# NekoImageLand/retto

Measured on AMD Instinct MI355X. Metric: images/sec end-to-end PP-OCRv4 det+rec @960x960, higher is better.
Workload: dtype f32

## Files before the change

### include/retto_hip.h

```cpp
#ifndef RETTO_HIP_H
#define RETTO_HIP_H

#include <stddef.h>
#include <stdint.h>

#ifdef __cplusplus
extern "C" {
#endif

#define RT_API __attribute__((visibility("default")))

typedef enum rt_status {
  RT_OK = 0,
  RT_ERR_IO = 1,
  RT_ERR_IMAGE = 2,
  RT_ERR_SHAPE = 3,
  RT_ERR_BACKEND = 4,
  RT_ERR_UTF8 = 5,
  RT_ERR_MODEL_NOT_FOUND = 7,
  RT_ERR_INVALID = 8,
  RT_ERR_CAPACITY = 9
} rt_status;

typedef struct rt_model_source {
// ... 69 lines not shown
                        int mem, const float* const* det_map_override, rt_results** out);
typedef void (*rt_stage_callback)(void* user, int page, int stage, const char* json);
RT_API int rt_run_batch_stream(rt_session* s, const uint8_t* const* rgb, const int* hs, const int* ws, int n_pages,
                               int mem, const float* const* det_map_override, rt_stage_callback cb, void* user,
                               rt_results** out);
#define RT_MAX_INFLIGHT 8
typedef struct rt_ticket rt_ticket;
RT_API int rt_submit_batch(rt_session* s, const uint8_t* const* rgb, const int* hs, const int* ws, int n_pages, int mem,
                           const float* const* det_map_override, rt_ticket** out);
RT_API int rt_wait_batch(rt_session* s, rt_ticket* ticket, rt_results** out);
RT_API void rt_results_free(rt_results* r);
RT_API int rt_results_pages(const rt_results* r);
RT_API int rt_results_count(const rt_results* r, int page);
RT_API const float* rt_results_boxes(const rt_results* r, int page);
RT_API const float* rt_results_det_scores(const rt_results* r, int page);
RT_API const uint16_t* rt_results_cls_labels(const rt_results* r, int page);
RT_API const float* rt_results_cls_scores(const rt_results* r, int page);
RT_API const float* rt_results_rec_scores(const rt_results* r, int page);
RT_API int rt_results_rec_tokens(const rt_results* r, int page, int line, const int32_t** tokens);
RT_API const char* rt_results_rec_text(const rt_results* r, int page, int line);
RT_API double rt_results_det_checksum(const rt_results* r);
RT_API const char* rt_results_json(rt_results* r, int page, int stage);

RT_API int rt_device_malloc(rt_session* s, size_t bytes, void** out);
RT_API int rt_device_free(rt_session* s, void* p);
RT_API int rt_memcpy_h2d(rt_session* s, void* dst, const void* src, size_t bytes);
RT_API int rt_memcpy_d2h(rt_session* s, void* dst, const void* src, size_t bytes);
RT_API int rt_synchronize(rt_session* s);
RT_API int rt_set_lanes(rt_session* s, int lanes);
RT_API int rt_profile_enable(rt_session* s, int on);
RT_API int rt_profile_get(rt_session* s, const char* const** names, const float** ms, const int** calls, int* n);

RT_API int rt_onnx_to_rtwb(int which, const void* onnx, size_t len, void** out, size_t* out_len, char* err, size_t err_cap);
RT_API void rt_buffer_free(void* p);

RT_API int rt_host_cpu_budget(void);
RT_API int rt_decode_image(const void* data, size_t len, uint8_t** rgb, int* h, int* w, char* err, size_t err_cap);
RT_API int rt_run_encoded_batch(rt_session* s, const void* const* files, const size_t* lens, int n_pages,
                                rt_stage_callback cb, void* user, rt_results** out);
RT_API int rt_parse_dictionary(const void* data, size_t len, char** out, size_t* out_len, int* n_entries, char* err, size_t err_cap);
RT_API int rt_format_f32(float v, char* buf, size_t cap);
RT_API size_t rt_model_manifest(int which, char* buf, size_t cap);

RT_API int rt_rccl_unique_id(void* id, size_t cap, char* err, size_t err_cap);
RT_API int rt_broadcast_blobs(const void* id, int rank, int world, int device_id, int root, int n_blobs, void** data, size_t* lens,
                              char* err, size_t err_cap);

RT_API void rt_debug_set_variants(int gemm_variant, int dw_variant, int flags);
RT_API int rt_debug_conv16(rt_session* s, const float* x, int n, int cin, int h, int w, const float* wt, int cout, int kh, int kw,
                           int sh, int sw, const float* bias, int act, float* out);
RT_API int rt_bench_gemm(rt_session* s, long long M, int K, int N, int variant, int iters, float* ms_out, float* maxdiff_out);
RT_API int rt_bench_gemm_err(rt_session* s, long long M, int K, int N, int variant, int rows, int act, unsigned seed, double* out4);
RT_API int rt_bench_lc(rt_session* s, int n, int h, int w, int cin, int cout, int stride, int form, int iters, float* ms_out, float* maxdiff_out);

#ifdef __cplusplus
}
#endif
#endif
```

### retto_amd/_lib.py

```python
from __future__ import annotations

import ctypes as C
import os

_HERE = os.path.dirname(os.path.abspath(__file__))
LIB_PATH = os.path.join(_HERE, "libretto_hip.so")

RT_OK = 0
RT_MEM_HOST, RT_MEM_DEVICE, RT_MEM_HOST_MAPS_DEVICE = 0, 1, 2
RT_MAX_INFLIGHT = 8
RT_DTYPE_F32, RT_DTYPE_F16 = 0, 1
STATUS_NAMES = {0: "OK", 1: "IOError", 2: "ImageError", 3: "ShapeError", 4: "BackendError", 5: "Utf8Error",
                7: "ModelNotFoundError", 8: "InvalidArgument", 9: "CapacityError"}


class ModelSource(C.Structure):
    _fields_ = [("path", C.c_char_p), ("data", C.c_void_p), ("len", C.c_size_t)]


class Config(C.Structure):
    _fields_ = [
        ("struct_size", C.c_uint32), ("device_id", C.c_int32),
        ("det", ModelSource), ("cls", ModelSource), ("rec", ModelSource), ("dict", ModelSource),
        ("max_side_len", C.c_int32), ("min_side_len", C.c_int32),
        ("det_limit_side_len", C.c_int32), ("det_limit_type", C.c_int32),
        ("det_mean", C.c_float * 3), ("det_std", C.c_float * 3), ("det_scale", C.c_float),
        ("det_thresh", C.c_float), ("det_box_thresh", C.c_float), ("det_unclip_ratio", C.c_float),
        ("det_min_mini_box_size", C.c_int32), ("det_dilation", C.c_int32),
        ("cls_image_shape", C.c_int32 * 3), ("cls_batch_num", C.c_int32), ("cls_thresh", C.c_float),
        ("rec_image_shape", C.c_int32 * 3), ("rec_batch_num", C.c_int32),
        ("max_boxes_per_page", C.c_int32), ("det_sub_batch", C.c_int32), ("lanes", C.c_int32), ("dtype", C.c_int32),
    ]


EXPORTS = [
    "rt_config_default", "rt_create", "rt_destroy", "rt_last_error", "rt_version",
    "rt_det", "rt_cls", "rt_rec", "rt_rec_ragged", "rt_rec_classes", "rt_model_info",
    "rt_resize_both_dims", "rt_resize_both", "rt_det_input_dims", "rt_det_preprocess", "rt_det_postprocess",
    "rt_crop_dims", "rt_crop_images", "rt_scale_and_clip", "rt_resize_norm_width", "rt_resize_norm_image",
    "rt_ctc_decode",
    "rt_run_batch", "rt_run_batch_stream", "rt_submit_batch", "rt_wait_batch", "rt_host_cpu_budget", "rt_results_free", "rt_results_pages", "rt_results_count", "rt_results_boxes",
    "rt_results_det_scores", "rt_results_cls_labels", "rt_results_cls_scores", "rt_results_rec_scores",
    "rt_results_rec_tokens", "rt_results_rec_text", "rt_results_det_checksum", "rt_results_json",
    "rt_device_malloc", "rt_device_free", "rt_memcpy_h2d", "rt_memcpy_d2h", "rt_synchronize",
    "rt_set_lanes", "rt_profile_enable", "rt_profile_get",
    "rt_onnx_to_rtwb", "rt_buffer_free", "rt_model_manifest", "rt_decode_image", "rt_run_encoded_batch",
    "rt_debug_set_variants", "rt_bench_gemm", "rt_bench_gemm_err", "rt_bench_lc", "rt_debug_conv16", "rt_parse_dictionary", "rt_format_f32", "rt_rccl_unique_id", "rt_broadcast_blobs",
]

STAGE_CALLBACK = C.CFUNCTYPE(None, C.c_void_p, C.c_int, C.c_int, C.c_char_p)

_lib = None


def source_digest() -> str:
    import glob
    import hashlib
    h = hashlib.sha256()
    files = sorted(glob.glob(os.path.join(_HERE, "csrc", "*.hip")) + glob.glob(os.path.join(_HERE, "csrc", "*.cpp")) +
                   glob.glob(os.path.join(_HERE, "csrc", "*.h")) + [os.path.join(os.path.dirname(_HERE), "include", "retto_hip.h")])
    for f in files:
        h.update(os.path.basename(f).encode()); h.update(open(f, "rb").read())
    return h.hexdigest()[:16]


def load():
    global _lib
    if _lib is not None:
        return _lib
    if not os.path.exists(LIB_PATH):
        raise ImportError(
            f"{LIB_PATH} is missing: build it with `make -C retto_amd/csrc` (python -c 'import __graft_entry__ as g; "
            "g.build()'). retto_amd has no CPU fallback.")
    lib = C.CDLL(LIB_PATH)
    P = C.POINTER
    lib.rt_last_error.restype = C.c_char_p
    lib.rt_last_error.argtypes = [C.c_void_p]
    lib.rt_version.restype = C.c_char_p
    lib.rt_create.argtypes = [P(Config), P(C.c_void_p)]
    lib.rt_destroy.argtypes = [C.c_void_p]
    lib.rt_destroy.restype = None
    lib.rt_results_free.argtypes = [C.c_void_p]
    lib.rt_results_free.restype = None
    lib.rt_results_boxes.restype = P(C.c_float)
    lib.rt_results_det_scores.restype = P(C.c_float)
    lib.rt_results_cls_labels.restype = P(C.c_uint16)
    lib.rt_results_cls_scores.restype = P(C.c_float)
    lib.rt_results_rec_scores.restype = P(C.c_float)
    lib.rt_results_rec_text.restype = C.c_char_p
    lib.rt_results_json.restype = C.c_char_p
    lib.rt_results_det_checksum.restype = C.c_double
    for name in ("rt_results_boxes", "rt_results_det_scores", "rt_results_cls_labels", "rt_results_cls_scores",
                 "rt_results_rec_scores", "rt_results_count"):
        getattr(lib, name).argtypes = [C.c_void_p, C.c_int]
    lib.rt_results_pages.argtypes = [C.c_void_p]
    lib.rt_results_det_checksum.argtypes = [C.c_void_p]
    lib.rt_results_rec_tokens.argtypes = [C.c_void_p, C.c_int, C.c_int, P(P(C.c_int32))]
    lib.rt_results_rec_text.argtypes = [C.c_void_p, C.c_int, C.c_int]
    lib.rt_results_json.argtypes = [C.c_void_p, C.c_int, C.c_int]
    lib.rt_scale_and_clip.argtypes = [C.c_void_p, C.c_int, C.c_double, C.c_double, C.c_double, C.c_double]
# ... 43 lines not shown
```

### retto_amd/csrc/api.cpp

```cpp
#include <thread>
#include <sched.h>
#include <atomic>
#include <cmath>
#include <cstdio>
#include <cstdlib>
#include <cstring>
#include <new>

#include "geom_math.h"
#include "session.h"
#include "onnx_import.h"
#include "image_decode.h"

using namespace rt;

static thread_local std::string g_create_error;
static void capture_variant_defaults();
const char* rt_results_json_impl(rt_results* r, int page, int stage);

static void quiesce(rt_session* s) {
  if (!s) return;
  (void)hipSetDevice(s->device);
  if (s->st) (void)hipStreamSynchronize(s->st);
  for (auto& h : s->helpers)
// ... 613 lines not shown
    float *dx = bufs.alloc<float>(nin), *dwd = bufs.alloc<float>(hwd.size()), *dbd = bufs.alloc<float>(hbd.size()), *dw = bufs.alloc<float>(hw.size()),
          *db = bufs.alloc<float>(hb.size()), *dy = bufs.alloc<float>(nout), *dy0 = bufs.alloc<float>(nout);
    ImgGeom *dgi = bufs.alloc<ImgGeom>(n), *dgo = bufs.alloc<ImgGeom>(n);
    RT_HIP_CHECK(hipMemset(dy, 0, nout * 4)); RT_HIP_CHECK(hipMemset(dy0, 0, nout * 4));
    RT_HIP_CHECK(hipMemcpy(dx, hx.data(), nin * 4, hipMemcpyHostToDevice)); RT_HIP_CHECK(hipMemcpy(dwd, hwd.data(), hwd.size() * 4, hipMemcpyHostToDevice));
    RT_HIP_CHECK(hipMemcpy(dbd, hbd.data(), hbd.size() * 4, hipMemcpyHostToDevice)); RT_HIP_CHECK(hipMemcpy(dw, hw.data(), hw.size() * 4, hipMemcpyHostToDevice));
    RT_HIP_CHECK(hipMemcpy(db, hb.data(), hb.size() * 4, hipMemcpyHostToDevice));
    RT_HIP_CHECK(hipMemcpy(dgi, gi.data(), n * sizeof(ImgGeom), hipMemcpyHostToDevice)); RT_HIP_CHECK(hipMemcpy(dgo, go.data(), n * sizeof(ImgGeom), hipMemcpyHostToDevice));
    Epilogue e; e.bias = db; e.act = ACT_HSWISH; e.has_lab = 1; e.lab_a = 1.01f; e.lab_c = 0.02f;
    const int dw_act = (sh == 2 && sw == 2) ? ACT_NONE : ACT_HSWISH, dw_lab = !(sh == 2 && sw == 2);
    float* dy1 = nullptr;
    auto run = [&](float* out) {
      if (nn::g_lc_wave == 0 && !nn::lc_thin_supported(3, sh, sw, Cp, cin, Np)) {
        if (!dy1) dy1 = bufs.alloc<float>((size_t)n * ho * wo * Cp);
        nn::dwconv(s->st, 3, sh, sw, dx, dgi, dgo, n, ho, wo, Cp, cin, dwd, dbd, dw_act, dw_lab, 0.99f, 0.01f, dy1, nullptr);
        nn::gemm(s->st, dy1, Cp, (long long)n * ho * wo, Cp, dw, cout, Np, out, ldy, 0, e);
        return;
      }
      nn::lc_thin(s->st, sh, sw, dx, dgi, dgo, n, ho, wo, Cp, cin, dwd, dbd, dw_act, dw_lab, 0.99f, 0.01f, dw, cout, Np, out, ldy, e);
    };
    nn::g_lc_wave = getenv("RT_BENCH_LC_REF") ? atoi(getenv("RT_BENCH_LC_REF")) : 0; run(dy0);
    nn::g_lc_wave = form; run(dy);
    Events ev; RT_HIP_CHECK(hipEventCreate(&ev.a)); RT_HIP_CHECK(hipEventCreate(&ev.b));
    hipEvent_t a = ev.a, b = ev.b;
    RT_HIP_CHECK(hipEventRecord(a, s->st));
    for (int i = 0; i < iters; i++) run(dy);
    RT_HIP_CHECK(hipEventRecord(b, s->st));
    RT_HIP_CHECK(hipStreamSynchronize(s->st));
    float ms = 0; RT_HIP_CHECK(hipEventElapsedTime(&ms, a, b)); *ms_out = ms / iters;
    if (maxdiff_out) {
      const size_t cnt = std::min<size_t>(nout, (size_t)1 << 22);
      std::vector<float> c0(cnt), c1(cnt);
      float md = 0;
      for (size_t off : {(size_t)0, nout - cnt}) {
        RT_HIP_CHECK(hipMemcpy(c0.data(), dy0 + off, cnt * 4, hipMemcpyDeviceToHost)); RT_HIP_CHECK(hipMemcpy(c1.data(), dy + off, cnt * 4, hipMemcpyDeviceToHost));
        size_t bad = 0;
        std::map<std::string, int> hist;
        for (size_t i = 0; i < cnt; i++) {
          const float d = std::fabs(c0[i] - c1[i]); md = (d > md || d != d) ? (d != d ? INFINITY : d) : md;
          if (d != 0 && getenv("RT_BENCH_LC_DUMP")) {
            const size_t e = off + i, px = e / ldy; const int ch = (int)(e % ldy), img = (int)(px / ((size_t)ho * wo)), yy = (int)(px % ((size_t)ho * wo)) / wo, xx = (int)(px % wo);
            if (bad++ < 4) fprintf(stderr, "  diff img %d y %d x %d ch %d: %g vs %g\n", img, yy, xx, ch, c0[i], c1[i]);
            hist["x%16=" + std::to_string(xx % 16)]++; hist["ch%4=" + std::to_string(ch % 4)]++; hist["ch/16=" + std::to_string(ch / 16)]++; hist["y%2=" + std::to_string(yy % 2)]++;
            hist["tx=" + std::to_string(xx / 16)]++; hist["q=" + std::to_string((ch % 16) / 4)]++;
          }
        }
        if (bad) { fprintf(stderr, "  %zu of %zu differ:", bad, cnt); for (auto& kv : hist) fprintf(stderr, " %s:%d", kv.first.c_str(), kv.second); fprintf(stderr, "\n"); }
      }
      *maxdiff_out = md;
    }
  });
}

}
```

### retto_amd/csrc/nn.h

```cpp
#pragma once
#include "common.h"

namespace rt {
namespace nn {

constexpr int KC = 32;

void gemm(hipStream_t st, const float* A, int lda, long long M, int K, const float* Wp, int N, int Npad16, float* C,
          int ldc, int coff, const Epilogue& epi);
const char* gemm_pw_label(long long M, int Npad16, bool a_scale = false, int se_tile_rows = 0);
bool gemm_w_supported(int lda, long long M, int K, int N, int Npad16, const Epilogue& epi, int ldc = 0, int coff = 0);
void gemm_w(hipStream_t st, const float* A, int lda, long long M, int K, const float* Wp, int N, int Npad16, float* C, int ldc, int coff,
            const Epilogue& epi);
bool gemm_dma_supported(int lda, long long M, int K, int N, int Npad16, const Epilogue& epi);
void gemm_dma(hipStream_t st, const float* A, int lda, long long M, int K, const float* Wp, int N, int Npad16, float* C,
              int ldc, int coff, const Epilogue& epi);
extern int g_gemm_split;
bool gemm_split_supported(int lda, long long M, int K, int N, int Npad16, const Epilogue& epi);
void gemm_split(hipStream_t st, const float* A, int lda, long long M, int K, const float* Wp, int N, int Npad16, float* C,
                int ldc, int coff, const Epilogue& epi);
void gemm_split_forget(const float* Wp);
void set_dw_xcd(int v);
extern int g_dw_wide_slab_min, g_dw_wide3_min, g_dw_wide_lp;
extern int g_dw_variant;
extern int g_gemm_variant;
extern int g_gemm_dma;
extern int g_dw_sweep;

bool conv13_flat_supported(int N, int Npad16);
void conv13_flat(hipStream_t st, const float* x, int ldx, long long rows, const unsigned char* flags, int Cin, const float* Wp, int N,
                 int Npad16, float* y, int ldy, const Epilogue& epi);
void conv_sp(hipStream_t st, int KH, int KW, const float* x, int ldx, const ImgGeom* geom, int n_img, int maxH,
             int maxW, int Cin, const float* Wp, int N, int Npad16, float* y, int ldy, const Epilogue& epi);

void dwconv(hipStream_t st, int K, int sh, int sw, const float* x, const ImgGeom* gin, const ImgGeom* gout, int n_img,
            int maxHo, int maxWo, int Cp, int C, const float* Wd, const float* bias, int act, int has_lab,
            float lab_a, float lab_c, float* y, float* pool = nullptr);
void dwconv_pool_layout(int K, int sh, int sw, int Cp, int maxHo, int maxWo, int* chunks, int* strip_R, int* strips_per_block);
void se_fc_from_dw(hipStream_t st, const float* partial, const ImgGeom* geom, int n_img, int chunks, int strip_R,
                   int strips_per_block, int C, int Cp, const float* w1, const float* b1, const float* w2, const float* b2,
                   int Cr, float slope, int residual, float* scale);
int gemm_tile_rows(long long M, int Npad16);
int gemm_se_tile_rows(int lda, long long M, int K, int N, int Npad16, int act, long long min_pix);
extern int g_argmax_wide;
int gemm_argmax_tiles(int Npad16);
void argmax_merge(hipStream_t st, const float* pm, const int* pi, const float* ps, int tiles, long long rows, int* idx,
                  float* prob);

extern int g_cls_fused;
bool cls_block_supported(int k, int sh, int sw, int cin, int mid, int cout, int act, int maxH_in, int maxW, int max_pix_out);
void cls_block(hipStream_t st, int k, int sh, bool se, int act, const float* x, const ImgGeom* gin, const ImgGeom* gout, int n_img,
               int maxH_in, int maxW, int max_pix_out, int cin, int mid, int mid_cp, int cout, const float* Wexp, const float* bexp,
               const float* Wdw, const float* bdw, const float* w1, const float* b1, const float* w2, const float* b2, int cr, float slope,
               const float* Wlin, const float* blin, bool shortcut, float* y, float* dscr);
extern int g_lc_thin;
bool lc_thin_supported(int K, int sh, int sw, int Cp, int C, int Npad16);
void lc_thin(hipStream_t st, int sh, int sw, const float* x, const ImgGeom* gin, const ImgGeom* gout, int n_img, int maxHo,
             int maxWo, int Cp, int C, const float* Wd, const float* bd, int dw_act, int dw_has_lab, float dw_a, float dw_c,
             const float* Wp, int N, int Npad16, float* y, int ldy, const Epilogue& epi);
extern int g_lc_wave;
bool lc_block_supported(int K, int sh, int sw, int Cp, int C, int N, int Npad16, int dw_act, int dw_has_lab, const Epilogue& epi,
                        int maxHo, int maxWo);
bool lc_wave_supported(int K, int sh, int sw, int Cp, int C, int N, int Npad16, int dw_act, int dw_has_lab, const Epilogue& epi);
void lc_wave(hipStream_t st, int sh, int sw, const float* x, const ImgGeom* gin, const ImgGeom* gout, int n_img, int maxHo,
             int maxWo, int Cp, int C, const float* Wd, const float* bd, int dw_act, int dw_has_lab, float dw_a, float dw_c,
             const float* Wp, int N, int Npad16, float* y, int ldy, const Epilogue& epi);

struct U8Page { const uint8_t* rgb; long long npix; long long out_pix; };
void stem_conv_u8(hipStream_t st, const U8Page* pages, float scale, const float* mean3, const float* std3, const ImgGeom* gin,
                  const ImgGeom* gout, int n_img, int maxHo, int maxWo, int COUT, const float* Ws, const float* bias, int act,
                  float* y);
void stem_conv(hipStream_t st, const float* x, const ImgGeom* gin, const ImgGeom* gout, int n_img, int maxHo, int maxWo,
               int COUT, const float* Ws, const float* bias, int act, float* y);

void nchw3_to_nhwc4(hipStream_t st, const float* in, int n, int H, int W, float* out);

int pool_chunks(long long max_pix);
void se_scale(hipStream_t st, const float* x, const ImgGeom* geom, int n_img, long long max_pix, int C, int Cp,
              const float* w1, const float* b1, const float* w2, const float* b2, int Cr, float slope, int residual,
              float* partial, float* scale);
// ... 62 lines not shown
```

### retto_amd/csrc/nn_kernels.hip

```cpp
#include "nn.h"
#include "nn_dev.h"

#include <algorithm>
#include <cstdlib>

namespace rt {
namespace nn {

constexpr int LROW = KC + 4;

template <int NT>
__device__ __forceinline__ void mma_chunk(const float* __restrict__ xs0, const float* __restrict__ xs1,
                                          const float* __restrict__ ws, int nt_valid, f32x4 (&acc)[2][NT], int r,
                                          int q) {
#pragma unroll
  for (int g = 0; g < KC / 16; g++) {
    f32x4 a0 = *reinterpret_cast<const f32x4*>(xs0 + g * 16 + 4 * q);
    f32x4 a1 = *reinterpret_cast<const f32x4*>(xs1 + g * 16 + 4 * q);
#pragma unroll
    for (int nt = 0; nt < NT; nt++) {
      if (nt < nt_valid) {
        f32x4 b = *reinterpret_cast<const f32x4*>(ws + (nt * 16 + r) * LROW + g * 16 + 4 * q);
#pragma unroll
        for (int s = 0; s < 4; s++) {
// ... 1227 lines not shown
#pragma unroll
      for (int dx = 0; dx < K; dx++) {
        const f32x4 w = *reinterpret_cast<const f32x4*>(wl + ((dy * K + dx) * LP + c4) * 4);
#pragma unroll
        for (int j = 0; j < 4; j++)
#pragma unroll
          for (int e = 0; e < 4; e++) acc[r][j][e] = fmaf(v[j * SW + dx][e], w[e], acc[r][j][e]);
      }
    }
  }
  f32x4 ps = {0.f, 0.f, 0.f, 0.f};
  act_dispatch(act, has_lab, false, [&](auto at, auto lt, auto) {
    constexpr int A = decltype(at)::value, L = decltype(lt)::value;
#pragma unroll
    for (int r = 0; r < R; r++) {
      const int oy = oy0 + r;
      if (oy >= go.H) break;
#pragma unroll
      for (int j = 0; j < 4; j++) {
        if (ox0 + j >= go.W) break;
        f32x4 o;
#pragma unroll
        for (int e = 0; e < 4; e++) {
          const float t = epi_val<A, L>(acc[r][j][e], act, has_lab, lab_a, lab_c);
          o[e] = (ch + e < C) ? t : 0.f;
        }
        *reinterpret_cast<f32x4*>(y + (go.off + (long long)oy * go.W + ox0 + j) * Cp + ch) = o;
        if (POOL) ps += o;
      }
    }
  });
  psum = ps;
  } else {
    psum = f32x4{0.f, 0.f, 0.f, 0.f};
  }
  if (POOL) {
    __shared__ __attribute__((aligned(16))) float red[4 * LP * 4];
#pragma unroll
    for (int d = LP; d < 64; d <<= 1)
#pragma unroll
      for (int e = 0; e < 4; e++) psum[e] += __shfl_xor(psum[e], d);
    if ((tid & 63) < LP) *reinterpret_cast<f32x4*>(red + ((tid >> 6) * LP + (tid & (LP - 1))) * 4) = psum;
    __syncthreads();
    if (tid < LP && cbase + tid * 4 < Cp) {
      f32x4 t = *reinterpret_cast<const f32x4*>(red + tid * 4);
#pragma unroll
      for (int w = 1; w < 4; w++) t += *reinterpret_cast<const f32x4*>(red + (w * LP + tid) * 4);
      *reinterpret_cast<f32x4*>(pool + ((long long)by * nbx + bx) * Cp + cbase + tid * 4) = t;
    }
  }
}

typedef unsigned u32x4 __attribute__((ext_vector_type(4)));
template <int K, int LP, int PX, int WAVES>
__global__ __launch_bounds__(256, WAVES) void k_dwconv_sweep(const float* __restrict__ x, const ImgGeom* __restrict__ gin,
                                                           const ImgGeom* __restrict__ gout, int Cp, int C,
                                                           const float* __restrict__ Wd, const float* __restrict__ bias, int act,
                                                           int has_lab, float lab_a, float lab_c, float* __restrict__ y) {
  constexpr int NV = PX - 1 + K, P = K / 2, SPB = 256 / LP;
  __shared__ __attribute__((aligned(16))) float wl[K * K * LP * 4];
  const ImgGeom gi = gin[blockIdx.y], go = gout[blockIdx.y];
  const int strips_x = (go.W + PX - 1) / PX;
  if ((int)blockIdx.x * SPB >= strips_x) return;
  const int cbase = blockIdx.z * LP * 4;
  const int tid = threadIdx.x;
  for (int i = tid; i < K * K * LP; i += 256) {
    int t = i / LP, cc = i % LP;
    f32x4 v = {0.f, 0.f, 0.f, 0.f};
    if (cbase + cc * 4 < Cp) v = *reinterpret_cast<const f32x4*>(Wd + t * Cp + cbase + cc * 4);
    *reinterpret_cast<f32x4*>(wl + i * 4) = v;
  }
  __syncthreads();
  const int c4 = tid % LP, ch = cbase + c4 * 4;
  const int strip = (int)blockIdx.x * SPB + tid / LP;
  if (ch >= Cp || strip >= strips_x) return;
  const int ox0 = strip * PX, H = gi.H;
  const f32x4 b = *reinterpret_cast<const f32x4*>(bias + ch);
  f32x4 acc[K][PX];
#pragma unroll
  for (int r = 0; r < K; r++)
#pragma unroll
    for (int j = 0; j < PX; j++) acc[r][j] = b;
  unsigned loff[NV];
#pragma unroll
  for (int j = 0; j < NV; j++) loff[j] = ox0 - P + j >= 0 ? (unsigned)((ox0 - P + j) * Cp + ch) * 4u : 0x80000000u;
  auto uni_ptr = [](const float* p_) {
    const unsigned long long v = (unsigned long long)p_;
    const unsigned lo = __builtin_amdgcn_readfirstlane((unsigned)v), hi = __builtin_amdgcn_readfirstlane((unsigned)(v >> 32));
    return (float*)(((unsigned long long)hi << 32) | lo);
  };
  const float* xim = uni_ptr(x + gi.off * Cp);
  float* yim = uni_ptr(y + go.off * Cp);
  const unsigned row_bytes = (unsigned)__builtin_amdgcn_readfirstlane(gi.W * Cp * 4);
  act_dispatch(act, has_lab, false, [&](auto at, auto lt, auto) {
    constexpr int A = decltype(at)::value, L = decltype(lt)::value;
    auto store_row = [&](int oy, f32x4 (&a)[PX]) __attribute__((always_inline)) {
      const __amdgpu_buffer_rsrc_t yrs = __builtin_amdgcn_make_buffer_rsrc(yim + (long long)oy * go.W * Cp, 0, row_bytes, 0x00020000);
#pragma unroll
      for (int j = 0; j < PX; j++) {
        f32x4 o;
#pragma unroll
        for (int e = 0; e < 4; e++) {
          const float t = epi_val<A, L>(a[j][e], act, has_lab, lab_a, lab_c);
          o[e] = (ch + e < C) ? t : 0.f;
        }
        __builtin_amdgcn_raw_buffer_store_b128(__builtin_bit_cast(u32x4, o), yrs, loff[j + P], 0, 0);
        a[j] = b;
      }
    };
    for (int i0 = 0; i0 < H; i0 += K) {
#pragma unroll
      for (int u = 0; u < K; u++) {
        const int i = i0 + u;
        if (i < H) {
          const __amdgpu_buffer_rsrc_t xrs = __builtin_amdgcn_make_buffer_rsrc(const_cast<float*>(xim) + (long long)i * gi.W * Cp, 0, row_bytes, 0x00020000);
          f32x4 v[NV];
#pragma unroll
          for (int j = 0; j < NV; j++) v[j] = __builtin_bit_cast(f32x4, __builtin_amdgcn_raw_buffer_load_b128(xrs, loff[j], 0, 0));
#pragma unroll
          for (int dy = 0; dy < K; dy++) {
            const int r = i + P - dy;
            const int slot = (u + P - dy + K) % K;
            if (r >= 0 && r < H) {
#pragma unroll
              for (int dx = 0; dx < K; dx++) {
                const f32x4 w = *reinterpret_cast<const f32x4*>(wl + ((dy * K + dx) * LP + c4) * 4);
#pragma unroll
                for (int j = 0; j < PX; j++)
#pragma unroll
                  for (int e = 0; e < 4; e++) acc[slot][j][e] = fmaf(v[j + dx][e], w[e], acc[slot][j][e]);
              }
            }
          }
          if (i - P >= 0) store_row(i - P, acc[(u - P + K) % K]);
        }
      }
    }
#pragma unroll
    for (int t = 0; t < P; t++) {
      const int r = H - P + t;
      if (r >= 0) {
#pragma unroll
        for (int sl = 0; sl < K; sl++)
          if (r % K == sl) store_row(r, acc[sl]);
      }
    }
  });
}

void set_dw_xcd(int v) { RT_HIP_CHECK(hipMemcpyToSymbol(HIP_SYMBOL(g_dw_xcd_dev), &v, sizeof(int))); }
int g_dw_wide_slab_min = 192;
static int dw_lanes_per_pixel(int K, int sh, int sw, int R, int Cp, bool pool);
int g_dw_wide3_min = 128;
int g_dw_wide_lp = 16;
int g_dw_variant = 0;
int g_dw_sweep = getenv("RT_DW_SWEEP") ? atoi(getenv("RT_DW_SWEEP")) : 4;
static int dw_strip_rows(int sh, int maxHo) {
  if (g_dw_variant == 4) return 2;
  if (maxHo == 6 || (maxHo == 3 && sh == 1)) return 3;
  return sh == 1 ? 4 : 2;
}

void dwconv(hipStream_t st, int K, int sh, int sw, const float* x, const ImgGeom* gin, const ImgGeom* gout, int n_img,
            int maxHo, int maxWo, int Cp, int C, const float* Wd, const float* bias, int act, int has_lab, float lab_a,
            float lab_c, float* y, float* pool) {
  if (n_img <= 0) return;
  if ((K == 3 || K == 5) && sh >= 1 && sh <= 2 && sw >= 1 && sw <= 2 && (g_dw_variant == 0 || g_dw_variant == 4)) {
    const int R = dw_strip_rows(sh, maxHo);
    long long strips = (long long)((maxWo + 3) / 4) * ((maxHo + R - 1) / R);
    const int lp = dw_lanes_per_pixel(K, sh, sw, R, Cp, pool != nullptr);
    if (g_dw_sweep && K == 5 && sh == 1 && sw == 1 && !pool && lp == 16 && maxHo >= 5 && maxHo <= 24) {
      const int spb = 256 / 16, px = g_dw_sweep == 4 ? 4 : 2;
      dim3 grids((unsigned)(((maxWo + px - 1) / px + spb - 1) / spb), n_img, (Cp + 63) / 64);
      if (px == 4) RT_LAUNCH((k_dwconv_sweep<5, 16, 4, 3>), grids, dim3(256), 0, st, x, gin, gout, Cp, C, Wd, bias, act, has_lab, lab_a, lab_c, y);
      else if (g_dw_sweep == 3) RT_LAUNCH((k_dwconv_sweep<5, 16, 2, 5>), grids, dim3(256), 0, st, x, gin, gout, Cp, C, Wd, bias, act, has_lab, lab_a, lab_c, y);
      else RT_LAUNCH((k_dwconv_sweep<5, 16, 2, 4>), grids, dim3(256), 0, st, x, gin, gout, Cp, C, Wd, bias, act, has_lab, lab_a, lab_c, y);
      return;
    }
    if (g_dw_sweep && K == 3 && sh == 1 && sw == 1 && !pool && lp == 16 && maxHo >= 3 && maxHo <= 24) {
      const int spb = 256 / 16;
      dim3 grids((unsigned)(((maxWo + 3) / 4 + spb - 1) / spb), n_img, (Cp + 63) / 64);
      RT_LAUNCH((k_dwconv_sweep<3, 16, 4, 4>), grids, dim3(256), 0, st, x, gin, gout, Cp, C, Wd, bias, act, has_lab, lab_a, lab_c, y);
      return;
    }
    if (lp != 8) {
      const int spb = 256 / lp;
      dim3 gridw((unsigned)((strips + spb - 1) / spb), n_img, (Cp + lp * 4 - 1) / (lp * 4));
#define RT_DWW(KK, RR, SH_, SW_, LL)                                                                                         \
  do {                                                                                                                       \
    if (pool) RT_LAUNCH((k_dwconv_rows<KK, RR, SH_, SW_, 1, LL>), gridw, dim3(256), 0, st, x, gin, gout, Cp, C, Wd, bias, act, has_lab, lab_a, lab_c, y, pool); \
    else RT_LAUNCH((k_dwconv_rows<KK, RR, SH_, SW_, 0, LL>), gridw, dim3(256), 0, st, x, gin, gout, Cp, C, Wd, bias, act, has_lab, lab_a, lab_c, y, pool); \
  } while (0)
#define RT_DWW_L(KK, RR, SH_, SW_) do { if (lp == 16) RT_DWW(KK, RR, SH_, SW_, 16); else RT_DWW(KK, RR, SH_, SW_, 32); } while (0)
      if (K == 5 && sh == 1 && sw == 1 && R == 4) { RT_DWW_L(5, 4, 1, 1); return; }
      if (K == 5 && sh == 1 && sw == 1 && R == 3) { RT_DWW_L(5, 3, 1, 1); return; }
      if (K == 5 && sh == 2 && sw == 1 && R == 2) { RT_DWW_L(5, 2, 2, 1); return; }
      if (K == 5 && sh == 2 && sw == 1 && R == 3) { RT_DWW_L(5, 3, 2, 1); return; }
      if (K == 5 && sh == 2 && sw == 2 && R == 2) { RT_DWW_L(5, 2, 2, 2); return; }
      if (K == 3 && sh == 1 && sw == 1 && R == 4 && !pool) { RT_DWW(3, 4, 1, 1, 16); return; }
      if (K == 3 && sh == 1 && sw == 2 && R == 4 && !pool) { RT_DWW(3, 4, 1, 2, 16); return; }
#undef RT_DWW_L
#undef RT_DWW
      throw RtError(8, "dwconv: no wide-slab instantiation for a shape dw_lanes_per_pixel() lists");
    }
    dim3 grid((unsigned)((strips + 31) / 32), n_img, (Cp + 31) / 32);
#define RT_DWR(KK, RR, SH_, SW_)                                                                                              \
  do {                                                                                                                       \
    if (pool) RT_LAUNCH((k_dwconv_rows<KK, RR, SH_, SW_, 1>), grid, dim3(256), 0, st, x, gin, gout, Cp, C, Wd, bias, act, has_lab, lab_a, lab_c, y, pool); \
    else RT_LAUNCH((k_dwconv_rows<KK, RR, SH_, SW_, 0>), grid, dim3(256), 0, st, x, gin, gout, Cp, C, Wd, bias, act, has_lab, lab_a, lab_c, y, pool); \
  } while (0)
    const int code = (K == 5 ? 4 : 0) + (sh == 2 ? 2 : 0) + (sw == 2 ? 1 : 0);
#define RT_DWR_R(KK, SH_, SW_, RBIG) \
  do { if (R == 3) RT_DWR(KK, 3, SH_, SW_); else if (R == RBIG) RT_DWR(KK, RBIG, SH_, SW_); else RT_DWR(KK, 2, SH_, SW_); } while (0)
    switch (code) {
      case 0: RT_DWR_R(3, 1, 1, 4); break; case 1: RT_DWR_R(3, 1, 2, 4); break;
      case 2: RT_DWR_R(3, 2, 1, 2); break; case 3: RT_DWR_R(3, 2, 2, 2); break;
      case 4: RT_DWR_R(5, 1, 1, 4); break; case 5: RT_DWR_R(5, 1, 2, 4); break;
      case 6: RT_DWR_R(5, 2, 1, 2); break; default: RT_DWR_R(5, 2, 2, 2); break;
    }
#undef RT_DWR_R
#undef RT_DWR
    return;
  }
  throw RtError(8, "dwconv: unsupported kernel size / stride");
}

template <int COUT>
__global__ __launch_bounds__(256) void k_stem(const float* __restrict__ x, const ImgGeom* __restrict__ gin,
                                              const ImgGeom* __restrict__ gout, const float* __restrict__ Ws,
                                              const float* __restrict__ bias, int act, float* __restrict__ y) {
  __shared__ float w[27 * COUT + COUT];
  for (int i = threadIdx.x; i < 27 * COUT; i += 256) w[i] = Ws[i];
  for (int i = threadIdx.x; i < COUT; i += 256) w[27 * COUT + i] = bias[i];
  __syncthreads();
  const ImgGeom gi = gin[blockIdx.y], go = gout[blockIdx.y];
  long long p = (long long)blockIdx.x * 256 + threadIdx.x;
  if (p >= (long long)go.H * go.W) return;
// ... 1160 lines not shown
```

Measured before the change: 1092.

## Extend depthwise sweep kernel to strided and pooled variants

Generalizes the row-sweep depthwise conv kernel to handle vertical stride 2, horizontal stride 2, and a fused SE-style pooling reduction through shared memory. New dispatch paths send 5x5 stride-2x1, pooled 5x5 stride-1, and 3x3 stride-1x2 layers (mainly in the recognition model) to the sweep kernel instead of the strip-tiled k_dwconv_rows kernel. The aim is to reuse input rows across output rows with rolling accumulators and less redundant loading. A gating env var controls the forms, and a benchmark/validation entry point is added. The risks are correctness of the pooled partial layout and added register pressure.

```diff
diff --git a/include/retto_hip.h b/include/retto_hip.h
--- a/include/retto_hip.h
+++ b/include/retto_hip.h
@@ -145,6 +145,8 @@
 RT_API int rt_bench_gemm(rt_session* s, long long M, int K, int N, int variant, int iters, float* ms_out, float* maxdiff_out);
 RT_API int rt_bench_gemm_err(rt_session* s, long long M, int K, int N, int variant, int rows, int act, unsigned seed, double* out4);
 RT_API int rt_bench_lc(rt_session* s, int n, int h, int w, int cin, int cout, int stride, int form, int iters, float* ms_out, float* maxdiff_out);
+RT_API int rt_bench_dwconv(rt_session* s, int n, int h, int w, int c, int k, int stride, int pool, int variant, int iters, float* ms_out,
+                           float* maxdiff_out);
 
 #ifdef __cplusplus
 }
diff --git a/retto_amd/_lib.py b/retto_amd/_lib.py
--- a/retto_amd/_lib.py
+++ b/retto_amd/_lib.py
@@ -45,7 +45,7 @@
     "rt_device_malloc", "rt_device_free", "rt_memcpy_h2d", "rt_memcpy_d2h", "rt_synchronize",
     "rt_set_lanes", "rt_profile_enable", "rt_profile_get",
     "rt_onnx_to_rtwb", "rt_buffer_free", "rt_model_manifest", "rt_decode_image", "rt_run_encoded_batch",
-    "rt_debug_set_variants", "rt_bench_gemm", "rt_bench_gemm_err", "rt_bench_lc", "rt_debug_conv16", "rt_parse_dictionary", "rt_format_f32", "rt_rccl_unique_id", "rt_broadcast_blobs",
+    "rt_debug_set_variants", "rt_bench_gemm", "rt_bench_gemm_err", "rt_bench_lc", "rt_bench_dwconv", "rt_debug_conv16", "rt_parse_dictionary", "rt_format_f32", "rt_rccl_unique_id", "rt_broadcast_blobs",
 ]
 
 STAGE_CALLBACK = C.CFUNCTYPE(None, C.c_void_p, C.c_int, C.c_int, C.c_char_p)
diff --git a/retto_amd/csrc/api.cpp b/retto_amd/csrc/api.cpp
--- a/retto_amd/csrc/api.cpp
+++ b/retto_amd/csrc/api.cpp
@@ -689,4 +689,71 @@
   });
 }
 
-}
+RT_API int rt_bench_dwconv(rt_session* s, int n, int h, int w, int c, int k, int stride, int pool, int variant, int iters, float* ms_out,
+                           float* maxdiff_out) {
+  RT_REQUIRE(s && ms_out && n > 0 && h > 0 && w > 0 && c > 0 && (k == 3 || k == 5) && (stride == 11 || stride == 21 || stride == 12 || stride == 22) &&
+             iters >= 0, s, "rt_bench_dwconv: bad argument");
+  return guarded(s, [&] {
+    RT_HIP_CHECK(hipSetDevice(s->device));
+    capture_variant_defaults();
+    const int sh = stride / 10, sw = stride % 10, Cp = chan_pitch(c), ho = (h + sh - 1) / sh;
+    std::vector<ImgGeom> gi(n), go(n);
+    long long pin = 0, pout = 0;
+    int maxWo = 0;
+    for (int i = 0; i < n; i++) {
+      const int wi = std::max(1, w - (37 * i) % (w / 2 + 1)), wo = (wi + sw - 1) / sw;
+      gi[i] = ImgGeom{pin, h, wi, 0}; go[i] = ImgGeom{pout, ho, wo, 0};
+      pin += (long long)h * wi; pout += (long long)ho * wo; maxWo = std::max(maxWo, wo);
+    }
+    const size_t nin = (size_t)pin * Cp, nout = (size_t)pout * Cp;
+    int chunks = 0, strip_R = 0, spb = 0;
+    if (pool) nn::dwconv_pool_layout(k, sh, sw, Cp, ho, maxWo, &chunks, &strip_R, &spb);
+    const size_t npool = pool ? (size_t)n * chunks * Cp : 0;
+    std::vector<float> hx(nin), hwd((size_t)k * k * Cp), hbd(Cp);
+    uint32_t st = 4242;
+    auto rnd = [&]() { st = st * 1664525u + 1013904223u; return ((st >> 8) & 0xffff) / 32768.0f - 1.0f; };
+    for (auto& v : hx) v = rnd();
+    for (auto& v : hwd) v = rnd() * 0.3f;
+    for (auto& v : hbd) v = rnd() * 0.1f;
+    DevBufs bufs;
+    RestoreInt keep_sweep(nn::g_dw_sweep), keep_forms(nn::g_dw_sweep_forms);
+    float *dx = bufs.alloc<float>(nin), *dwd = bufs.alloc<float>(hwd.size()), *dbd = bufs.alloc<float>(hbd.size()), *dy = bufs.alloc<float>(nout),
+          *dy0 = bufs.alloc<float>(nout), *dp = pool ? bufs.alloc<float>(npool) : nullptr, *dp0 = pool ? bufs.alloc<float>(npool) : nullptr;
+    ImgGeom *dgi = bufs.alloc<ImgGeom>(n), *dgo = bufs.alloc<ImgGeom>(n);
+    RT_HIP_CHECK(hipMemset(dy, 0xff, nout * 4)); RT_HIP_CHECK(hipMemset(dy0, 0xff, nout * 4));
+    if (pool) { RT_HIP_CHECK(hipMemset(dp, 0xff, npool * 4)); RT_HIP_CHECK(hipMemset(dp0, 0xff, npool * 4)); }
+    RT_HIP_CHECK(hipMemcpy(dx, hx.data(), nin * 4, hipMemcpyHostToDevice)); RT_HIP_CHECK(hipMemcpy(dwd, hwd.data(), hwd.size() * 4, hipMemcpyHostToDevice));
+    RT_HIP_CHECK(hipMemcpy(dbd, hbd.data(), hbd.size() * 4, hipMemcpyHostToDevice));
+    RT_HIP_CHECK(hipMemcpy(dgi, gi.data(), n * sizeof(ImgGeom), hipMemcpyHostToDevice)); RT_HIP_CHECK(hipMemcpy(dgo, go.data(), n * sizeof(ImgGeom), hipMemcpyHostToDevice));
+    auto run = [&](float* out, float* pl) {
+      nn::dwconv(s->st, k, sh, sw, dx, dgi, dgo, n, ho, maxWo, Cp, c, dwd, dbd, ACT_HSWISH, 1, 0.99f, 0.01f, out, pl);
+    };
+    nn::g_dw_sweep = 0; run(dy0, dp0);
+    nn::g_dw_sweep = variant < 0 ? 0 : g_default_dw_sweep;
+    nn::g_dw_sweep_forms = variant < 0 ? 0 : variant;
+    run(dy, dp);
+    Events ev; RT_HIP_CHECK(hipEventCreate(&ev.a)); RT_HIP_CHECK(hipEventCreate(&ev.b));
+    RT_HIP_CHECK(hipEventRecord(ev.a, s->st));
+    for (int i = 0; i < iters; i++) run(dy, dp);
+    RT_HIP_CHECK(hipEventRecord(ev.b, s->st));
+    RT_HIP_CHECK(hipStreamSynchronize(s->st));
+    float ms = 0; RT_HIP_CHECK(hipEventElapsedTime(&ms, ev.a, ev.b)); *ms_out = iters > 0 ? ms / iters : 0.f;
+    if (maxdiff_out) {
+      float md = 0;
+      auto cmp = [&](const float* a_d, const float* b_d, size_t cnt) {
+        std::vector<float> a(cnt), b(cnt);
+        RT_HIP_CHECK(hipMemcpy(a.data(), a_d, cnt * 4, hipMemcpyDeviceToHost)); RT_HIP_CHECK(hipMemcpy(b.data(), b_d, cnt * 4, hipMemcpyDeviceToHost));
+        for (size_t i = 0; i < cnt; i++) {
+          if (memcmp(&a[i], &b[i], 4) == 0) continue;
+          const float d = std::fabs(a[i] - b[i]);
+          md = d != d ? INFINITY : std::max(md, d > 0 ? d : 1e-45f);
+        }
+      };
+      cmp(dy0, dy, nout);
+      if (pool) cmp(dp0, dp, npool);
+      *maxdiff_out = md;
+    }
+  });
+}
+
+}
diff --git a/retto_amd/csrc/nn.h b/retto_amd/csrc/nn.h
--- a/retto_amd/csrc/nn.h
+++ b/retto_amd/csrc/nn.h
@@ -26,6 +26,7 @@
 extern int g_gemm_variant;
 extern int g_gemm_dma;
 extern int g_dw_sweep;
+extern int g_dw_sweep_forms;
 
 bool conv13_flat_supported(int N, int Npad16);
 void conv13_flat(hipStream_t st, const float* x, int ldx, long long rows, const unsigned char* flags, int Cin, const float* Wp, int N,
diff --git a/retto_amd/csrc/nn_kernels.hip b/retto_amd/csrc/nn_kernels.hip
--- a/retto_amd/csrc/nn_kernels.hip
+++ b/retto_amd/csrc/nn_kernels.hip
@@ -1303,13 +1303,20 @@
 }
 
 typedef unsigned u32x4 __attribute__((ext_vector_type(4)));
-template <int K, int LP, int PX, int WAVES>
+template <int K, int LP, int PX, int WAVES, int SH = 1, int SW = 1, int POOL = 0>
 __global__ __launch_bounds__(256, WAVES) void k_dwconv_sweep(const float* __restrict__ x, const ImgGeom* __restrict__ gin,
                                                            const ImgGeom* __restrict__ gout, int Cp, int C,
                                                            const float* __restrict__ Wd, const float* __restrict__ bias, int act,
-                                                           int has_lab, float lab_a, float lab_c, float* __restrict__ y) {
-  constexpr int NV = PX - 1 + K, P = K / 2, SPB = 256 / LP;
+                                                           int has_lab, float lab_a, float lab_c, float* __restrict__ y,
+                                                           float* __restrict__ pool, int pool_R, int pool_nbx) {
+  constexpr int NV = SW * (PX - 1) + K, P = K / 2, SPB = 256 / LP;
+  constexpr int NS = SH == 1 ? K : (K + SH - 1) / SH;
+  constexpr int G = SH * NS;
+  constexpr int NTAIL = (P + SH - 1) / SH;
+  constexpr int SYMAX = 4;
+  static_assert(!POOL || PX == 4, "pooled sweep: a thread column must be one k_dwconv_rows strip wide");
   __shared__ __attribute__((aligned(16))) float wl[K * K * LP * 4];
+  __shared__ __attribute__((aligned(16))) f32x4 pls[POOL ? SYMAX * SPB * LP : 1];
   const ImgGeom gi = gin[blockIdx.y], go = gout[blockIdx.y];
   const int strips_x = (go.W + PX - 1) / PX;
   if ((int)blockIdx.x * SPB >= strips_x) return;
@@ -1321,20 +1328,26 @@
     if (cbase + cc * 4 < Cp) v = *reinterpret_cast<const f32x4*>(Wd + t * Cp + cbase + cc * 4);
     *reinterpret_cast<f32x4*>(wl + i * 4) = v;
   }
-  __syncthreads();
   const int c4 = tid % LP, ch = cbase + c4 * 4;
   const int strip = (int)blockIdx.x * SPB + tid / LP;
-  if (ch >= Cp || strip >= strips_x) return;
-  const int ox0 = strip * PX, H = gi.H;
+  if (POOL) {
+#pragma unroll
+    for (int k = 0; k < SYMAX; k++) pls[(k * SPB + tid / LP) * LP + c4] = f32x4{0.f, 0.f, 0.f, 0.f};
+  }
+  __syncthreads();
+  const bool active = ch < Cp && strip < strips_x;
+  if (!POOL && !active) return;
+  if (active) {
+  const int ox0 = strip * PX, H = gi.H, Ho = go.H;
   const f32x4 b = *reinterpret_cast<const f32x4*>(bias + ch);
-  f32x4 acc[K][PX];
-#pragma unroll
-  for (int r = 0; r < K; r++)
+  f32x4 acc[NS][PX];
+#pragma unroll
+  for (int r = 0; r < NS; r++)
 #pragma unroll
     for (int j = 0; j < PX; j++) acc[r][j] = b;
   unsigned loff[NV];
 #pragma unroll
-  for (int j = 0; j < NV; j++) loff[j] = ox0 - P + j >= 0 ? (unsigned)((ox0 - P + j) * Cp + ch) * 4u : 0x80000000u;
+  for (int j = 0; j < NV; j++) loff[j] = ox0 * SW - P + j >= 0 ? (unsigned)((ox0 * SW - P + j) * Cp + ch) * 4u : 0x80000000u;
   auto uni_ptr = [](const float* p_) {
     const unsigned long long v = (unsigned long long)p_;
     const unsigned lo = __builtin_amdgcn_readfirstlane((unsigned)v), hi = __builtin_amdgcn_readfirstlane((unsigned)(v >> 32));
@@ -1343,10 +1356,17 @@
   const float* xim = uni_ptr(x + gi.off * Cp);
   float* yim = uni_ptr(y + go.off * Cp);
   const unsigned row_bytes = (unsigned)__builtin_amdgcn_readfirstlane(gi.W * Cp * 4);
+  const unsigned orow_bytes = SW == 1 ? row_bytes : (unsigned)__builtin_amdgcn_readfirstlane(go.W * Cp * 4);
+  f32x4 ps = {0.f, 0.f, 0.f, 0.f};
+  auto load_row = [&](int i, f32x4 (&dst)[NV]) __attribute__((always_inline)) {
+    const __amdgpu_buffer_rsrc_t xrs = __builtin_amdgcn_make_buffer_rsrc(const_cast<float*>(xim) + (long long)i * gi.W * Cp, 0, row_bytes, 0x00020000);
+#pragma unroll
+    for (int j = 0; j < NV; j++) dst[j] = __builtin_bit_cast(f32x4, __builtin_amdgcn_raw_buffer_load_b128(xrs, loff[j], 0, 0));
+  };
   act_dispatch(act, has_lab, false, [&](auto at, auto lt, auto) {
     constexpr int A = decltype(at)::value, L = decltype(lt)::value;
     auto store_row = [&](int oy, f32x4 (&a)[PX]) __attribute__((always_inline)) {
-      const __amdgpu_buffer_rsrc_t yrs = __builtin_amdgcn_make_buffer_rsrc(yim + (long long)oy * go.W * Cp, 0, row_bytes, 0x00020000);
+      const __amdgpu_buffer_rsrc_t yrs = __builtin_amdgcn_make_buffer_rsrc(yim + (long long)oy * go.W * Cp, 0, orow_bytes, 0x00020000);
 #pragma unroll
       for (int j = 0; j < PX; j++) {
         f32x4 o;
@@ -1355,48 +1375,69 @@
           const float t = epi_val<A, L>(a[j][e], act, has_lab, lab_a, lab_c);
           o[e] = (ch + e < C) ? t : 0.f;
         }
-        __builtin_amdgcn_raw_buffer_store_b128(__builtin_bit_cast(u32x4, o), yrs, loff[j + P], 0, 0);
+        const unsigned soff = SW == 1 ? loff[j + P] : (unsigned)((ox0 + j) * Cp + ch) * 4u;
+        __builtin_amdgcn_raw_buffer_store_b128(__builtin_bit_cast(u32x4, o), yrs, soff, 0, 0);
+        if (POOL && ox0 + j < go.W) ps += o;
         a[j] = b;
       }
+      if (POOL && (oy % pool_R == pool_R - 1 || oy == Ho - 1)) {
+        pls[((oy / pool_R) * SPB + tid / LP) * LP + c4] = ps;
+        ps = f32x4{0.f, 0.f, 0.f, 0.f};
+      }
     };
-    for (int i0 = 0; i0 < H; i0 += K) {
-#pragma unroll
-      for (int u = 0; u < K; u++) {
+    for (int i0 = 0; i0 < H; i0 += G) {
+#pragma unroll
+      for (int u = 0; u < G; u++) {
         const int i = i0 + u;
         if (i < H) {
-          const __amdgpu_buffer_rsrc_t xrs = __builtin_amdgcn_make_buffer_rsrc(const_cast<float*>(xim) + (long long)i * gi.W * Cp, 0, row_bytes, 0x00020000);
           f32x4 v[NV];
-#pragma unroll
-          for (int j = 0; j < NV; j++) v[j] = __builtin_bit_cast(f32x4, __builtin_amdgcn_raw_buffer_load_b128(xrs, loff[j], 0, 0));
+          load_row(i, v);
 #pragma unroll
           for (int dy = 0; dy < K; dy++) {
-            const int r = i + P - dy;
-            const int slot = (u + P - dy + K) % K;
-            if (r >= 0 && r < H) {
+            if ((u + P - dy + G) % SH != 0) continue;
+            const int q = (u + P - dy + G) / SH - NS;
+            const int r = i0 / SH + q;
+            const int slot = (q + NS) % NS;
+            if (r >= 0 && r < Ho) {
 #pragma unroll
               for (int dx = 0; dx < K; dx++) {
                 const f32x4 w = *reinterpret_cast<const f32x4*>(wl + ((dy * K + dx) * LP + c4) * 4);
 #pragma unroll
                 for (int j = 0; j < PX; j++)
 #pragma unroll
-                  for (int e = 0; e < 4; e++) acc[slot][j][e] = fmaf(v[j + dx][e], w[e], acc[slot][j][e]);
+                  for (int e = 0; e < 4; e++) acc[slot][j][e] = fmaf(v[j * SW + dx][e], w[e], acc[slot][j][e]);
               }
             }
           }
-          if (i - P >= 0) store_row(i - P, acc[(u - P + K) % K]);
+          if ((u - P + G) % SH == 0 && i - P >= 0 && (i - P) / SH < Ho) store_row((i - P) / SH, acc[((u - P + G) / SH) % NS]);
         }
       }
     }
 #pragma unroll
-    for (int t = 0; t < P; t++) {
-      const int r = H - P + t;
-      if (r >= 0) {
-#pragma unroll
-        for (int sl = 0; sl < K; sl++)
-          if (r % K == sl) store_row(r, acc[sl]);
+    for (int t = 0; t < NTAIL; t++) {
+      const int r = Ho - NTAIL + t;
+      if (r >= 0 && r * SH + P >= H) {
+#pragma unroll
+        for (int sl = 0; sl < NS; sl++)
+          if (r % NS == sl) store_row(r, acc[sl]);
       }
     }
   });
+  }
+  if (POOL) {
+    __syncthreads();
+    const int sy = (go.H + pool_R - 1) / pool_R, bl = tid / LP;
+    if (bl < sy && cbase + c4 * 4 < Cp) {
+      const int bxr = (int)blockIdx.x * sy + bl;
+      if (bxr * SPB < strips_x * sy) {
+        auto part = [&](int s) { const int l = bl * SPB + s; return pls[((l % sy) * SPB + l / sy) * LP + c4]; };
+        f32x4 t = (part(0) + part(1)) + (part(2) + part(3));
+#pragma unroll
+        for (int w = 1; w < 4; w++) t += (part(4 * w) + part(4 * w + 1)) + (part(4 * w + 2) + part(4 * w + 3));
+        *reinterpret_cast<f32x4*>(pool + ((long long)blockIdx.y * pool_nbx + bxr) * Cp + ch) = t;
+      }
+    }
+  }
 }
 
 void set_dw_xcd(int v) { RT_HIP_CHECK(hipMemcpyToSymbol(HIP_SYMBOL(g_dw_xcd_dev), &v, sizeof(int))); }
@@ -1406,6 +1447,7 @@
 int g_dw_wide_lp = 16;
 int g_dw_variant = 0;
 int g_dw_sweep = getenv("RT_DW_SWEEP") ? atoi(getenv("RT_DW_SWEEP")) : 4;
+int g_dw_sweep_forms = getenv("RT_DW_SWEEP_FORMS") ? atoi(getenv("RT_DW_SWEEP_FORMS")) : 3;
 static int dw_strip_rows(int sh, int maxHo) {
   if (g_dw_variant == 4) return 2;
   if (maxHo == 6 || (maxHo == 3 && sh == 1)) return 3;
@@ -1420,20 +1462,42 @@
     const int R = dw_strip_rows(sh, maxHo);
     long long strips = (long long)((maxWo + 3) / 4) * ((maxHo + R - 1) / R);
     const int lp = dw_lanes_per_pixel(K, sh, sw, R, Cp, pool != nullptr);
-    if (g_dw_sweep && K == 5 && sh == 1 && sw == 1 && !pool && lp == 16 && maxHo >= 5 && maxHo <= 24) {
+#define RT_DWS(KK, PX_, WV, SH_, SW_, PL)                                                                                    \
+  RT_LAUNCH((k_dwconv_sweep<KK, 16, PX_, WV, SH_, SW_, PL>), grids, dim3(256), 0, st, x, gin, gout, Cp, C, Wd, bias, act, has_lab, \
+            lab_a, lab_c, y, pool, R, pool_nbx)
+    const int pool_nbx = (int)((strips + 15) / 16);
+    if (g_dw_sweep && K == 5 && sh == 1 && sw == 1 && !pool && lp == 16 && (maxHo >= 5 || ((g_dw_sweep_forms & 8) && maxHo >= 3)) && maxHo <= 24) {
       const int spb = 256 / 16, px = g_dw_sweep == 4 ? 4 : 2;
       dim3 grids((unsigned)(((maxWo + px - 1) / px + spb - 1) / spb), n_img, (Cp + 63) / 64);
-      if (px == 4) RT_LAUNCH((k_dwconv_sweep<5, 16, 4, 3>), grids, dim3(256), 0, st, x, gin, gout, Cp, C, Wd, bias, act, has_lab, lab_a, lab_c, y);
-      else if (g_dw_sweep == 3) RT_LAUNCH((k_dwconv_sweep<5, 16, 2, 5>), grids, dim3(256), 0, st, x, gin, gout, Cp, C, Wd, bias, act, has_lab, lab_a, lab_c, y);
-      else RT_LAUNCH((k_dwconv_sweep<5, 16, 2, 4>), grids, dim3(256), 0, st, x, gin, gout, Cp, C, Wd, bias, act, has_lab, lab_a, lab_c, y);
+      if (px == 4) RT_DWS(5, 4, 3, 1, 1, 0);
+      else if (g_dw_sweep == 3) RT_DWS(5, 2, 5, 1, 1, 0);
+      else RT_DWS(5, 2, 4, 1, 1, 0);
       return;
     }
     if (g_dw_sweep && K == 3 && sh == 1 && sw == 1 && !pool && lp == 16 && maxHo >= 3 && maxHo <= 24) {
       const int spb = 256 / 16;
       dim3 grids((unsigned)(((maxWo + 3) / 4 + spb - 1) / spb), n_img, (Cp + 63) / 64);
-      RT_LAUNCH((k_dwconv_sweep<3, 16, 4, 4>), grids, dim3(256), 0, st, x, gin, gout, Cp, C, Wd, bias, act, has_lab, lab_a, lab_c, y);
+      RT_DWS(3, 4, 4, 1, 1, 0);
       return;
     }
+    const bool sw_pool_ok = !pool || ((g_dw_sweep_forms & 2) && (maxHo + R - 1) / R <= 4);
+    if (g_dw_sweep && (g_dw_sweep_forms & 1) && K == 5 && sh == 2 && sw == 1 && lp == 16 && sw_pool_ok && maxHo >= 2 && maxHo <= 12) {
+      dim3 grids((unsigned)(((maxWo + 3) / 4 + 15) / 16), n_img, (Cp + 63) / 64);
+      if (pool) RT_DWS(5, 4, 4, 2, 1, 1);
+      else RT_DWS(5, 4, 4, 2, 1, 0);
+      return;
+    }
+    if (g_dw_sweep && K == 5 && sh == 1 && sw == 1 && pool && lp == 16 && sw_pool_ok && maxHo >= 5 && maxHo <= 24) {
+      dim3 grids((unsigned)(((maxWo + 3) / 4 + 15) / 16), n_img, (Cp + 63) / 64);
+      RT_DWS(5, 4, 3, 1, 1, 1);
+      return;
+    }
+    if (g_dw_sweep && (g_dw_sweep_forms & 4) && K == 3 && sh == 1 && sw == 2 && !pool && lp == 16 && maxHo >= 3 && maxHo <= 24) {
+      dim3 grids((unsigned)(((maxWo + 3) / 4 + 15) / 16), n_img, (Cp + 63) / 64);
+      RT_DWS(3, 4, 4, 1, 2, 0);
+      return;
+    }
+#undef RT_DWS
     if (lp != 8) {
       const int spb = 256 / lp;
       dim3 gridw((unsigned)((strips + spb - 1) / spb), n_img, (Cp + lp * 4 - 1) / (lp * 4));
```

Result: no change. 1102, median of 6 (+0.9%).
